# l13039968960/stm32H7-YOLO

Measured on AMD Instinct MI355X. Metric: images/sec int8 YOLO-face 56x56, higher is better.
Workload: dtype int8; 1 GPU; BASELINE configs[1]: batch=4096 int8 YOLO-face 56x56x3 frames per GPU, fused LDS-resident forward + GPU box decode; frames_per_gpu=4096, global_batch=4096, frame_bytes_in=9408, frame_bytes_out=882, input_batches_rotated=8, input_bytes_resident=308281344, kernel=yoloface56_fused<F=2,NW=8>, requant_rounding=ref, parallelism=single GPU, gather_every=1, collectives_issued=0, launch_streams=2

## Files before the change

stm32h7-yolo_amd/csrc/yf_kernels.hip.h:

```cpp
#include <hip/hip_runtime.h>
#include <stddef.h>
#include <stdint.h>
#include <type_traits>
#include "yf_tables.h"

#pragma clang diagnostic push
#pragma clang diagnostic ignored "-Wint-to-pointer-cast"
#if !defined(YF_LAB) || !defined(YF_LAUNDER)
#undef YF_LAUNDER
#define YF_LAUNDER 0
#endif
#define YF_ROW_SKEW 4
namespace YF_NS {

#ifndef YF_NOINLINE_STAGES
#define YF_STAGE_FN __device__ __forceinline__
#else
#define YF_STAGE_FN __device__ __attribute__((noinline))
#endif

typedef int v4i __attribute__((ext_vector_type(4)));
typedef short v2s __attribute__((ext_vector_type(2)));

#if !defined(YF_H0) || YF_H0 == 56
// ... 477 lines not shown
  for (int i = tid; i < F * IH * NCH * 5; i += NT) {
    const int cg = i % 5; int t = i / 5;
    const int k = t % NCH; t /= NCH;
    const int y = t % IH; const int f = t / IH;
    char* fbase = frames + f * B_T4::FS;
    const char* row = fbase + B_T4::at(y, 0) + 4 * cg;
    char* dst = fbase + B_HB::OFF + (y * OW) * 20 + 4 * cg;
    pool8_sweep<NO, B_T4::W - 1>(min(k * NO, OW - NO),
                                 [&](int x) { return lds_u32(row + x * B_T4::S); },
                                 [&](int ox, const SplitB& v) { *reinterpret_cast<uint32_t*>(dst + ox * 20) = v.merge(); });
  }
}
template <int F, int NT, bool STASH = false>
YF_STAGE_FN void pool8_v(char* frames, int tid) {
  constexpr int NO = 5, OW = B_HB::W, OH = B_T14::H, NCH = (OH + NO - 1) / NO;
  static_assert(OH >= NO, "column shorter than one sweep");
  for (int i = tid; i < F * OW * NCH * 5; i += NT) {
    const int cg = i % 5; int t = i / 5;
    const int k = t % NCH; t /= NCH;
    const int ox = t % OW; const int f = t / OW;
    char* fbase = frames + f * B_HB::FS;
    const char* col = fbase + B_HB::OFF + ox * 20 + 4 * cg;
    char* dst = fbase + B_T14::OFF + ox * B_T14::S + 4 * cg;
    pool8_sweep<NO, B_HB::H - 1>(min(k * NO, OH - NO),
                                 [&](int r) { return lds_u32(col + r * (OW * 20)); },
                                 [&](int oy, const SplitB& v) {
                                   *reinterpret_cast<uint32_t*>(dst + oy * (OW * B_T14::S)) = lut4_raw<YF_L_Q21>(v);
                                   if constexpr (STASH) *reinterpret_cast<uint32_t*>(dst + oy * (OW * B_T14::S) + YF_T14_CONV_BASE) = v.merge();
                                 });
  }
}

namespace v2 {
constexpr int LUT_B = YF_N_LUT * 256;
constexpr int JT = LUT_B, JT_B = 896;
constexpr int ZERO = JT + JT_B, ZERO_B = 640;
constexpr int SLOT0 = ZERO + ZERO_B, SLOT_B = 2816;
constexpr int slot(int cs) { return SLOT0 + (cs & 1) * SLOT_B; }
struct Lay56 {
  static constexpr int ZERO = v2::ZERO, JT = v2::JT, JT_BYTES = v2::JT_B;
  static constexpr int slot(int cs) { return v2::slot(cs); }
};
constexpr int max_block() { int m = 0; for (int i = 0; i < YF_N_CS; ++i) m = PLAN.vb_bytes[i] > m ? PLAN.vb_bytes[i] : m; return m; }
static_assert(max_block() <= SLOT_B && SLOT0 % 16 == 0 && SLOT_B % 16 == 0, "a constant block fits a ring slot");

typedef const __attribute__((address_space(3))) v4i* lds_v4i_ptr;
typedef const __attribute__((address_space(3))) v4u* lds_v4u_ptr;
typedef const __attribute__((address_space(3))) uint32_t* lds_u32_ptr;
typedef const __attribute__((address_space(3))) v2u* lds_u2_ptr;
__device__ __forceinline__ v4i lds_v4i(uint32_t a) { return *(lds_v4i_ptr)a; }
__device__ __forceinline__ v4u lds_v4u(uint32_t a) { return *(lds_v4u_ptr)a; }

template <int CS, class LAY = Lay56, int BYTES_ = -1>
__device__ __forceinline__ void fetch_consts(const uint8_t* __restrict__ tab, int wave, int lane) {
  constexpr int BYTES = BYTES_ >= 0 ? BYTES_ : PLAN.vb_bytes[CS], NCHUNK = (BYTES + 1023) / 1024;
  if (wave < NCHUNK) {
    asm volatile("" : "+v"(lane));
    const int off = wave * 1024 + lane * 16;
    if (off < BYTES) {
      const uint8_t* src = tab + PLAN.vb_off[CS] + off;
      const uint32_t dst = (uint32_t)(LAY::slot(CS) + wave * 1024);
      uint32_t keep;
      asm volatile("s_mov_b32 %0, m0\n\ts_mov_b32 m0, %2\n\ts_nop 0\n\tglobal_load_lds_dwordx4 %1, off\n\ts_mov_b32 m0, %0"
                   : "=&s"(keep) : "v"(src), "s"(dst) : "memory");
    }
  }
}

template <int W, int SH = (W > 32 ? 20 : 16)> struct DivW {
  static constexpr uint32_t M = ((1u << SH) + W - 1) / W;
  static constexpr bool ok() { for (uint32_t p = 0; p < 2048; ++p) if (((p * M) >> SH) != p / W) return false; return true; }
  static_assert(ok(), "multiply-shift division is exact on [0, 2048)");
  __device__ static __forceinline__ int div(int p) { return (int)(((uint32_t)p * M) >> SH); }
};

template <int EPI, int LUT_ID, int LA, int STASH_LUT = -1>
__device__ __forceinline__ void epilogue2(char* dstpix, const char* addpix, char* headpix, int chq, int hq, const int (&idx)[4], const AddK& ad,
                                          char* stashpix = nullptr) {
  if constexpr (EPI == EPI_LUT) {
    *reinterpret_cast<uint32_t*>(dstpix + chq) = join4(lutb<LUT_ID>(idx[0]), lutb<LUT_ID>(idx[1]), lutb<LUT_ID>(idx[2]), lutb<LUT_ID>(idx[3]));
    if constexpr (STASH_LUT >= 0) {
      if (stashpix) *reinterpret_cast<uint32_t*>(stashpix + chq) =
          join4(*(lds_u8_ptr)(uint32_t)(STASH_LUT + idx[0]), *(lds_u8_ptr)(uint32_t)(STASH_LUT + idx[1]),
                *(lds_u8_ptr)(uint32_t)(STASH_LUT + idx[2]), *(lds_u8_ptr)(uint32_t)(STASH_LUT + idx[3]));
    }
  } else if constexpr (EPI == EPI_RAW) {
    *reinterpret_cast<uint32_t*>(dstpix + chq) = join4(idx[0], idx[1], idx[2], idx[3]) ^ 0x80808080u;
  } else if constexpr (EPI == EPI_ADD) {
    typedef const __attribute__((address_space(3))) int* lds_i32_ptr;
    if (stashpix) *reinterpret_cast<uint32_t*>(stashpix + chq) = join4(idx[0], idx[1], idx[2], idx[3]) ^ 0x80808080u;
    const uint32_t o = lds_u32(addpix + chq) ^ 0x80808080u;
    v4i sum;
#pragma unroll
    for (int j = 0; j < 4; ++j)
      sum[j] = *(lds_i32_ptr)(uint32_t)(LA + 4 * ((o >> (8 * j)) & 255)) + *(lds_i32_ptr)(uint32_t)(LA + 1024 + 4 * idx[j]);
    int r[4];
    requant4<false>(sum, v4u{ad.mo2, ad.mo2, ad.mo2, ad.mo2}, v4u{ad.zro, ad.zro, ad.zro, ad.zro},
                    v4ul{ad.c64o, ad.c64o, ad.c64o, ad.c64o}, v4i{ad.rso, ad.rso, ad.rso, ad.rso}, r);
    *reinterpret_cast<uint32_t*>(dstpix + chq) = join4(r[0], r[1], r[2], r[3]) ^ 0x80808080u;
  } else {
    const uint32_t v = join4(idx[0], idx[1], idx[2], idx[3]) ^ 0x80808080u;
    uint16_t* dst = reinterpret_cast<uint16_t*>(headpix + hq);
    dst[0] = (uint16_t)v;
    if (hq + 2 < 18) dst[1] = (uint16_t)(v >> 16);
  }
}

template <int EPI, int LUT_ID, int LA>
__device__ __forceinline__ void epilogue2_half(char* dstpix, const char* addpix, int chq, const int (&idx)[2], const AddK& ad) {
  static_assert(EPI == EPI_LUT || EPI == EPI_RAW || EPI == EPI_ADD, "half passes: LUT, raw and residual-add epilogues");
  if constexpr (EPI == EPI_LUT) {
    *reinterpret_cast<uint32_t*>(dstpix + chq) = join2(lutb<LUT_ID>(idx[0]), lutb<LUT_ID>(idx[1]));
  } else if constexpr (EPI == EPI_RAW) {
    *reinterpret_cast<uint32_t*>(dstpix + chq) = join2(idx[0], idx[1]) ^ 0x8080u;
  } else {
    typedef const __attribute__((address_space(3))) int* lds_i32_ptr;
    const uint32_t o = lds_u32(addpix + chq) ^ 0x80808080u;
    v4i sum = {0, 0, 0, 0};
#pragma unroll
    for (int j = 0; j < 2; ++j)
      sum[j] = *(lds_i32_ptr)(uint32_t)(LA + 4 * ((o >> (8 * j)) & 255)) + *(lds_i32_ptr)(uint32_t)(LA + 1024 + 4 * idx[j]);
    int r[2];
    requant2<false>(sum, v4u{ad.mo2, ad.mo2, ad.mo2, ad.mo2}, v4u{ad.zro, ad.zro, ad.zro, ad.zro},
                    v4ul{ad.c64o, ad.c64o, ad.c64o, ad.c64o}, v4i{ad.rso, ad.rso, ad.rso, ad.rso}, r);
    *reinterpret_cast<uint32_t*>(dstpix + chq) = join2(r[0], r[1]) ^ 0x8080u;
  }
}
#if !defined(YF_LAB) || !defined(YF_CHUNK_UNROLL)
#undef YF_CHUNK_UNROLL
#define YF_CHUNK_UNROLL 0
#endif
#define YF_HALF_PASS 1

template <int F, int NW, int TPJ, int KS, int BW, class IN, class OUT, int OUT_CH0, int COUT, int EPI, int LUT_ID, class ADDB, int CS,
          int STASH_OFF = -1, int STASH_S = 0, int STASH_LUT = -1, class LAY = Lay56, int LA_ABS = -1>
YF_STAGE_FN void dense2_stage(char* frames, char* out_all, const uint8_t* __restrict__ tab, const AddK ad, int wave, int lane) {
  constexpr int NP = (COUT + 3) / 4, NCH = (NP + TPJ - 1) / TPJ;
  constexpr int P = IN::P, TOT = F * P;
  constexpr bool FRAME_TILES = P <= 64;
  constexpr int MT = FRAME_TILES ? F : (TOT + 63) / 64;
  constexpr int JOBS = NCH * MT, KROW = 16 * KS;
  constexpr int SLOT = LAY::slot(CS), WB = plan_wbytes(CS), PV = SLOT + WB, LA = LA_ABS >= 0 ? LA_ABS : PV + NP * (int)sizeof(yf_pass_v);
  static_assert(yf_cs_dense[CS] >= 0 && KROW == PLAN_KROW[yf_cs_dense[CS]] && NP == plan_passes(CS), "stage and constant block agree");
  static_assert((EPI == EPI_ADD) == (yf_cs_add[CS] >= 0), "residual-add tables travel with their stage");
  static_assert(OUT::P == P || EPI == EPI_HEAD || EPI == EPI_HEAD_LDS, "1x1 conv keeps the grid");
  static_assert(IN::FS == OUT::FS && IN::FS == ADDB::FS, "one frame stride per stage");
  static_assert(IN::S >= 16 * (KS - 1) + BW && (BW == 4 || BW == 8 || BW == 16), "the pixel vector must cover all k-steps");
  static_assert(IN::RS == IN::W && IN::PT == 0 && IN::PL == 0, "dense inputs are plain buffers");
  const int g = lane >> 4, c = lane & 15;
  const bool a_on = (c >> 2) == g;
  const uint32_t a_lane = a_on ? (uint32_t)(SLOT + (c & 3) * KROW) : (uint32_t)LAY::ZERO;
  const uint32_t a_step = a_on ? (uint32_t)(TPJ * 4 * KROW) : 0u;
  const uint8_t* sc = tab + PLAN.sb_off[CS];
  int in_c = 0, out_c = 0, add_c = 0, stash_c = 0;
  static_assert(STASH_OFF < 0 || EPI == EPI_ADD || (EPI == EPI_LUT && STASH_LUT >= 0), "a stash is the pre-add convolution output or a second LUT's view");
  if constexpr (FRAME_TILES) {
    const int p = min(lane, P - 1);
    in_c = IN::OFF + p * IN::S;
    if constexpr (EPI == EPI_HEAD || EPI == EPI_HEAD_LDS) out_c = p * 18;
    else if constexpr (OUT::RS == OUT::W && OUT::PT == 0 && OUT::PL == 0) out_c = OUT::OFF + p * OUT::S + OUT_CH0;
    else { const int y = DivW<OUT::W>::div(p); out_c = OUT::at(y, p - y * OUT::W) + OUT_CH0; }
    add_c = ADDB::OFF + p * ADDB::S;
    if constexpr (STASH_OFF >= 0) stash_c = STASH_OFF + p * STASH_S;
  }
  int j0, j1;
  job_range<JOBS, NW>(wave, j0, j1);
  auto run_chunk = [&](const int chunk, int mt, const int n) __attribute__((always_inline)) {
    v4i a[TPJ][KS];
    PassV pv[TPJ];
    PassS ksr[TPJ];
    const uint32_t a_addr = a_lane + (uint32_t)chunk * a_step;
#pragma unroll
    for (int t = 0; t < TPJ; ++t) {
      const int ps = chunk * TPJ + t;
#pragma unroll
      for (int ks = 0; ks < KS; ++ks) a[t][ks] = lds_v4i(a_addr + (uint32_t)(t * 4 * KROW + 16 * ks));
      pv[t].m2 = lds_v4u((uint32_t)(PV + ps * 32));
      pv[t].zr = lds_v4u((uint32_t)(PV + ps * 32 + 16));
      const uint8_t* s = sc + min(ps, NP - 1) * (int)sizeof(yf_pass_s);
      ksr[t] = PassS{*(cv4ul_ptr)(uintptr_t)s, *(cv4i_ptr)(uintptr_t)(s + 32)};
    }
    const int cq = chunk * TPJ * 4;
    const int out_cc = out_c + cq, add_cc = add_c + cq;
    for (int k = 0; k < n; ++k, ++mt) {
      const char* src; char* dstpix = nullptr; const char* addpix = nullptr; char* headpix = nullptr; char* stashpix = nullptr;
      if constexpr (FRAME_TILES) {
        char* fbase = frames + mt * IN::FS;
        src = fbase + in_c;
        dstpix = fbase + out_cc; addpix = fbase + add_cc;
        if constexpr (STASH_OFF >= 0) stashpix = fbase + stash_c + cq;
        if constexpr (EPI == EPI_HEAD) headpix = out_all + mt * OUT_FRAME_BYTES + out_c;
        if constexpr (EPI == EPI_HEAD_LDS) headpix = fbase + OUT::OFF + out_c;
      } else {
        const int q = min(mt * 64 + lane, TOT - 1);
        int f = 0;
#pragma unroll
        for (int i = 1; i < F; ++i) f += (q >= i * P) ? 1 : 0;
        const int p = q - f * P;
        char* fbase = frames + f * IN::FS;
        src = fbase + IN::OFF + p * IN::S;
        if constexpr (EPI == EPI_HEAD) headpix = out_all + f * OUT_FRAME_BYTES + p * 18;
        else if constexpr (EPI == EPI_HEAD_LDS) headpix = fbase + OUT::OFF + p * 18;
        else if constexpr (OUT::RS == OUT::W && OUT::PT == 0 && OUT::PL == 0) dstpix = fbase + cq + OUT::OFF + p * OUT::S + OUT_CH0;
        else { const int y = DivW<OUT::W>::div(p); dstpix = fbase + cq + OUT::at(y, p - y * OUT::W) + OUT_CH0; }
        if constexpr (EPI == EPI_ADD) addpix = fbase + cq + ADDB::OFF + p * ADDB::S;
        if constexpr (STASH_OFF >= 0) stashpix = fbase + cq + STASH_OFF + p * STASH_S;
      }
      v4i b[KS];
#pragma unroll
      for (int ks = 0; ks < KS - 1; ++ks) b[ks] = *reinterpret_cast<const v4i*>(src + 16 * ks);
      const char* last = src + 16 * (KS - 1);
      if constexpr (BW == 16) b[KS - 1] = *reinterpret_cast<const v4i*>(last);
      else if constexpr (BW == 8) { const int2 t2 = *reinterpret_cast<const int2*>(last); b[KS - 1] = v4i{t2.x, t2.y, any_value(), any_value()}; }
      else b[KS - 1] = v4i{*reinterpret_cast<const int*>(last), any_value(), any_value(), any_value()};
#pragma unroll
      for (int t = 0; t < TPJ; ++t) {
        const int ps = chunk * TPJ + t;
        if (ps < NP) {
          v4i acc = acc_init(pv[t].zr);
#pragma unroll
          for (int ks = 0; ks < KS; ++ks) acc = __builtin_amdgcn_mfma_i32_16x16x64_i8(a[t][ks], b[ks], acc, 0, 0, 0);
          constexpr bool HALF_L = YF_HALF_PASS && COUT % 4 == 2 && STASH_OFF < 0 && (EPI == EPI_LUT || EPI == EPI_RAW || EPI == EPI_ADD);
          const bool half = HALF_L && t == (NP - 1) % TPJ && ps == NP - 1;
          if (half) {
            if constexpr (HALF_L) {
              int idx2[2];
              requant2<true, DENSE_SIGNLESS, RQ_FP32>(acc, pv[t].m2, pv[t].zr, ksr[t].c64, ksr[t].rs, idx2);
              epilogue2_half<EPI, LUT_ID, LA>(dstpix, addpix, t * 4, idx2, ad);
            }
          } else {
            int idx[4];
            requant4<true, DENSE_SIGNLESS, RQ_FP32>(acc, pv[t].m2, pv[t].zr, ksr[t].c64, ksr[t].rs, idx);
            epilogue2<EPI, LUT_ID, LA, STASH_LUT>(dstpix, addpix, headpix, t * 4, ps * 4, idx, ad, stashpix);
          }
        }
      }
    }
  };
  if constexpr (NCH <= YF_CHUNK_UNROLL) {
#pragma unroll
    for (int chunk = 0; chunk < NCH; ++chunk) {
      const int lo = max(j0, chunk * MT), hi = min(j1, (chunk + 1) * MT);
      if (lo < hi) run_chunk(chunk, lo - chunk * MT, hi - lo);
    }
  } else {
    int chunk = (int)((uint32_t)j0 / (uint32_t)MT), mt = j0 - chunk * MT, left = j1 - j0;
    while (left > 0) {
      const int n = min(left, MT - mt);
      run_chunk(chunk, mt, n);
      left -= n; ++chunk; mt = 0;
    }
  }
}

template <int F, int NW, int CS, class IN = B_IN, class OUT = B_T1, class LAY = Lay56>
YF_STAGE_FN void conv1_2_stage(char* frames, const uint8_t* __restrict__ tab, int wave, int lane) {
  constexpr int P = OUT::P, W1 = OUT::W, RSW = IN::RS, TOT = F * P;
  constexpr int MT = (TOT + 63) / 64;
  constexpr int SLOT = LAY::slot(CS), WB = plan_wbytes(CS), PV = SLOT + WB;
  const int g = lane >> 4, c = lane & 15;
  const bool a_on = (c >> 2) == g;
  const uint32_t a_addr = a_on ? (uint32_t)(SLOT + (c & 3) * YF_CONV1_KROW) : (uint32_t)LAY::ZERO;
  const uint8_t* sc = tab + PLAN.sb_off[CS];
  v4i a[2][3];
  PassV pv[2];
#pragma unroll
  for (int ps = 0; ps < 2; ++ps) {
#pragma unroll
    for (int ks = 0; ks < 3; ++ks) a[ps][ks] = lds_v4i(a_addr + (uint32_t)(ps * 4 * YF_CONV1_KROW + 16 * ks));
    pv[ps].m2 = lds_v4u((uint32_t)(PV + ps * 32));
    pv[ps].zr = lds_v4u((uint32_t)(PV + ps * 32 + 16));
  }
  int j0, j1;
  job_range<MT, NW>(wave, j0, j1);
  const AddK ad = {};
  for (int mt = j0; mt < j1; ++mt) {
    const int q = min(mt * 64 + lane, TOT - 1);
    int f = 0;
#pragma unroll
    for (int i = 1; i < F; ++i) f += (q >= i * P) ? 1 : 0;
    const int p = q - f * P;
    const int oy = DivW<W1>::div(p), ox = p - oy * W1;
    char* fbase = frames + f * IN::FS;
    const uint32_t* src = reinterpret_cast<const uint32_t*>(fbase + IN::OFF) + (2 * oy * RSW + 2 * ox + 3);
    const v4i b0 = {(int)src[0], (int)src[1], (int)src[2], (int)src[RSW]};
    const v4i b1 = {(int)src[RSW + 1], (int)src[RSW + 2], (int)src[2 * RSW], (int)src[2 * RSW + 1]};
    const v4i b2 = {(int)src[2 * RSW + 2], any_value(), any_value(), any_value()};
    char* dstpix = fbase + OUT::at(oy, ox);
#pragma unroll
    for (int ps = 0; ps < 2; ++ps) {
      const uint8_t* s = sc + ps * (int)sizeof(yf_pass_s);
      const PassS k = PassS{*(cv4ul_ptr)(uintptr_t)s, *(cv4i_ptr)(uintptr_t)(s + 32)};
      v4i acc = acc_init(pv[ps].zr);
      acc = __builtin_amdgcn_mfma_i32_16x16x64_i8(a[ps][0], b0, acc, 0, 0, 0);
      acc = __builtin_amdgcn_mfma_i32_16x16x64_i8(a[ps][1], b1, acc, 0, 0, 0);
      acc = __builtin_amdgcn_mfma_i32_16x16x64_i8(a[ps][2], b2, acc, 0, 0, 0);
      int idx[4];
      requant4<true, DENSE_SIGNLESS, RQ_FP32>(acc, pv[ps].m2, pv[ps].zr, k.c64, k.rs, idx);
      epilogue2<EPI_LUT, YF_L_LEAKY2, 0>(dstpix, nullptr, nullptr, 4 * ps, 0, idx, ad);
    }
  }
}

template <int F, int STRIDE, int W, int H>
constexpr int dw_rows_per_lane() {
#if YF_H0 == 56
  return STRIDE == 1 && F == 2 && W == 28 && H == 28 ? 7 : STRIDE == 1 && F == 2 && W == 14 && H == 14 ? 2 : 1;
#else
  return 1;
#endif
}
template <int F, int STRIDE, class IN, class OUT>
struct DwGeo {
  static constexpr int W = OUT::W, H = OUT::H;
  static constexpr int R = dw_rows_per_lane<F, STRIDE, OUT::W, OUT::H>(), BR = 4 * R;
  static constexpr int FL = (W <= 8 && F % 2 == 0) ? 2 : 1;
  static constexpr int NSEG = (W + 15) / 16, NRB = (H + BR - 1) / BR, NFP = F / FL;
  static constexpr int JPG = NFP * NRB * NSEG;
  static_assert(OUT::RS == W && OUT::PT == 0 && OUT::PL == 0, "depthwise outputs are plain buffers");
  static_assert(IN::FS == OUT::FS, "one frame stride per stage");
  static_assert(H >= BR && (W >= 16 || W * FL <= 16), "tile shape");
  static_assert(R == 1 || (STRIDE == 1 && FL == 1), "row window: stride-1 stages, one frame per job");
  __device__ static __forceinline__ uint2 job(int jj) {
    const int fp = jj / (NRB * NSEG); int rem = jj - fp * (NRB * NSEG);
    const int rb = rem / NSEG, seg = rem - rb * NSEG;
    const int oy0 = min(rb * BR, H - BR);
    const int x0 = (W >= 16) ? min(seg * 16, W - 16) : 0;
    const int fb = fp * FL * IN::FS;
    return uint2{(uint32_t)(fb + IN::OFF + (oy0 * STRIDE) * IN::ROWB + x0 * STRIDE * IN::S), (uint32_t)(fb + OUT::OFF + (oy0 * W + x0) * OUT::S)};
  }
};
#if YF_H0 == 56
template <int F, bool BATCH>
struct JobTabs {
  typedef TailBufs<BATCH ? FRAME_STRIDE / 2 : FRAME_STRIDE> U;
  static constexpr int FT = BATCH ? 2 * F : F;
  static constexpr int JT_DW3 = 0;
  static constexpr int JT_DW10 = JT_DW3 + 8 * DwGeo<F, 1, B_T1, B_T2>::JPG;
  static constexpr int JT_DW15 = JT_DW10 + 8 * DwGeo<F, 2, B_T4, B_T6>::JPG;
  static constexpr int JT_DW27 = JT_DW15 + 8 * DwGeo<F, 1, B_T8, B_T9>::JPG;
  static constexpr int JT_DW32 = JT_DW27 + 8 * DwGeo<FT, 2, typename U::T15, typename U::T17>::JPG;
  static constexpr int END = JT_DW32 + 8 * DwGeo<FT, 1, typename U::T19, typename U::T20>::JPG;
  static_assert(END <= JT_B, "job tables fit");
};
#endif
template <class B, bool RING, int F>
struct HaloGeo {
  static constexpr int HR = B::H + B::PT + (RING ? 1 : 0), WR = B::RS;
  static constexpr int NPIX = RING ? (2 * WR + 2 * (HR - 2)) : (WR + HR - 1);
  static constexpr int N = F * NPIX;
  static_assert(B::S % 4 == 0 && B::OFF % 4 == 0 && B::FS % 4 == 0, "dword pixels");
  __device__ static __forceinline__ uint32_t entry(int i) {
    const int f = i / NPIX, k = i - f * NPIX;
    int r, c;
    if constexpr (RING) {
      if (k < WR) { r = 0; c = k; }
      else if (k < 2 * WR) { r = HR - 1; c = k - WR; }
      else { const int m = k - 2 * WR; r = 1 + (m >> 1); c = (m & 1) ? WR - 1 : 0; }
    } else {
      if (k < WR) { r = 0; c = k; } else { r = 1 + (k - WR); c = 0; }
    }
    return (uint32_t)(f * B::FS + B::OFF + r * B::ROWB + c * B::S);
  }
};
#if YF_H0 == 56
template <int F, bool BATCH>
struct HaloTabs {
  typedef TailBufs<BATCH ? FRAME_STRIDE / 2 : FRAME_STRIDE> U;
  static constexpr int FT = BATCH ? 2 * F : F;
  typedef HaloGeo<B_T1, true, F> G1; typedef HaloGeo<B_T4, false, F> G4; typedef HaloGeo<B_T8, true, F> G8;
  typedef HaloGeo<B_T15, false, F> G15; typedef HaloGeo<typename U::T19, true, FT> G19;
  static constexpr int H_T1 = 0, H_T4 = H_T1 + 2 * G1::N, H_T8 = H_T4 + 2 * G4::N, H_T15 = H_T8 + 2 * G8::N, H_T19 = H_T15 + 2 * G15::N;
  static constexpr int BYTES = (H_T19 + 2 * G19::N + 15) & ~15;
};
constexpr int HT = SLOT0 + 2 * SLOT_B;
template <int F, bool BATCH> constexpr int pre_bytes() { return HT + HaloTabs<F, BATCH>::BYTES; }
template <class G, int HOFF, int NT>
__device__ __forceinline__ void build_halotab(char* smem, int tid) {
  for (int i = tid; i < G::N; i += NT) *reinterpret_cast<uint16_t*>(smem + HT + HOFF + 2 * i) = (uint16_t)(G::entry(i) >> 2);
}
template <class B, class G, int HOFF>
YF_STAGE_FN void fill_halo_t(char* frames, int zp, int tid) {
  typedef const __attribute__((address_space(3))) uint16_t* lds_u16_ptr;
  if (tid < G::N) {
    const uint32_t v = (uint32_t)(zp & 255) * 0x01010101u;
    char* p = frames + 4u * (uint32_t)*(lds_u16_ptr)(uint32_t)(HT + HOFF + 2 * tid);
    if constexpr (B::S % 8 == 0 && B::OFF % 8 == 0 && B::FS % 8 == 0) {
#pragma unroll
      for (int d = 0; d < B::S / 8; ++d) *reinterpret_cast<uint2*>(p + 8 * d) = uint2{v, v};
    } else {
#pragma unroll
      for (int d = 0; d < B::S / 4; ++d) *reinterpret_cast<uint32_t*>(p + 4 * d) = v;
    }
  }
}
#endif

template <int F, int STRIDE, class IN, class OUT, int JTOFF, class LAY = Lay56>
__device__ __forceinline__ void fill_jobtab(char* smem, int tid) {
  typedef DwGeo<F, STRIDE, IN, OUT> G;
  static_assert(JTOFF % 8 == 0 && JTOFF + G::JPG * 8 <= LAY::JT_BYTES, "job table in bounds");
  if (tid < G::JPG) *reinterpret_cast<uint2*>(smem + LAY::JT + JTOFF + 8 * tid) = G::job(tid);
}

template <int F, int NW, int STRIDE, class IN, class OUT, int C, int LUT_ID, int CS, int JTOFF, class LAY = Lay56>
YF_STAGE_FN void dw2_stage(char* frames, const uint8_t* __restrict__ tab, int wave, int lane) {
  typedef DwGeo<F, STRIDE, IN, OUT> G;
  constexpr int W = G::W, FL = G::FL, JPG = G::JPG;
  constexpr int NG = (C + 3) / 4, JOBS = NG * JPG;
  constexpr int DROW = STRIDE * IN::ROWB;
  constexpr int TS = IN::S, TR = IN::ROWB;
  constexpr int SLOT = LAY::slot(CS);
  static_assert(yf_cs_dw[CS] >= 0 && NG == plan_passes(CS), "stage and constant block agree");
  const int g = lane >> 4, c = lane & 15;
  const int fl = (FL == 2) ? (c >> 3) : 0;
  const int xl = (FL == 2) ? min(c & 7, W - 1) : min(c, W - 1);
  const char* lane_in = frames + fl * IN::FS + g * G::R * DROW + xl * STRIDE * IN::S;
  char* lane_out = frames + fl * IN::FS + (g * G::R * W + xl) * OUT::S;
  const bool a_on = (c >> 2) == g;
  const uint32_t a_lane = a_on ? (uint32_t)(SLOT + 4 * (c & 3)) : (uint32_t)LAY::ZERO;
  const uint32_t a_step = a_on ? (uint32_t)YF_DWV_GROUP_BYTES : 0u;
  const uint8_t* sc = tab + PLAN.sb_off[CS];
  int j, j1;
  job_range<JOBS, NW>(wave, j, j1);
  int cg = (int)((uint32_t)j / (uint32_t)JPG), jj = j - cg * JPG, left = j1 - j;
  while (left > 0) {
    const uint32_t wa = a_lane + (uint32_t)cg * a_step;
    v4i a0, a1, a2 = {0, 0, 0, 0};
    a0 = v4i{(int)*(lds_u32_ptr)(wa), (int)*(lds_u32_ptr)(wa + 16), (int)*(lds_u32_ptr)(wa + 32), (int)*(lds_u32_ptr)(wa + 48)};
    a1 = v4i{(int)*(lds_u32_ptr)(wa + 64), (int)*(lds_u32_ptr)(wa + 80), (int)*(lds_u32_ptr)(wa + 96), (int)*(lds_u32_ptr)(wa + 112)};
    a2[0] = (int)*(lds_u32_ptr)(wa + 128);
    PassV pv;
    pv.m2 = lds_v4u((uint32_t)(SLOT + cg * YF_DWV_GROUP_BYTES + 144));
    pv.zr = lds_v4u((uint32_t)(SLOT + cg * YF_DWV_GROUP_BYTES + 160));
    const uint8_t* s = sc + cg * (int)sizeof(yf_pass_s);
    const PassS k = PassS{*(cv4ul_ptr)(uintptr_t)s, *(cv4i_ptr)(uintptr_t)(s + 32)};
    const char* lin = lane_in + 4 * cg;
    char* lout = lane_out + 4 * cg;
    auto entry = [&](int job) { return *(lds_u2_ptr)(uint32_t)(LAY::JT + JTOFF + 8 * min(job, JPG - 1)); };
    auto taps = [&](const v2u e, v4i& b0, v4i& b1, v4i& b2, char*& dst) {
      const char* src = lin + e[0];
      b0[0] = (int)lds_u32(src);               b0[1] = (int)lds_u32(src + TS);          b0[2] = (int)lds_u32(src + 2 * TS);
      b0[3] = (int)lds_u32(src + TR);          b1[0] = (int)lds_u32(src + TR + TS);     b1[1] = (int)lds_u32(src + TR + 2 * TS);
      b1[2] = (int)lds_u32(src + 2 * TR);      b1[3] = (int)lds_u32(src + 2 * TR + TS); b2[0] = (int)lds_u32(src + 2 * TR + 2 * TS);
      dst = lout + e[1];
    };
    auto conv = [&](const v4i& b0, const v4i& b1, const v4i& b2) {
      v4i acc = acc_init(pv.zr);
      acc = __builtin_amdgcn_mfma_i32_16x16x64_i8(a0, b0, acc, 0, 0, 0);
      acc = __builtin_amdgcn_mfma_i32_16x16x64_i8(a1, b1, acc, 0, 0, 0);
      return __builtin_amdgcn_mfma_i32_16x16x64_i8(a2, b2, acc, 0, 0, 0);
    };
    auto finish = [&](const v4i& acc, char* dst) {
      if (YF_HALF_PASS && C % 4 == 2 && cg == NG - 1) {
        int idx2[2];
        requant2<true, false, RQ_FP32>(acc, pv.m2, pv.zr, k.c64, k.rs, idx2);
        *reinterpret_cast<uint32_t*>(dst) = join2(lutb<LUT_ID>(idx2[0]), lutb<LUT_ID>(idx2[1]));
      } else {
        int idx[4];
        requant4<true, false, RQ_FP32>(acc, pv.m2, pv.zr, k.c64, k.rs, idx);
        *reinterpret_cast<uint32_t*>(dst) = join4(lutb<LUT_ID>(idx[0]), lutb<LUT_ID>(idx[1]), lutb<LUT_ID>(idx[2]), lutb<LUT_ID>(idx[3]));
      }
    };
    const int n = min(left, JPG - jj);
    if constexpr (G::R > 1) {
      const v4i ar[3] = {v4i{a0[0], a0[1], a0[2], 0}, v4i{a0[3], a1[0], a1[1], 0}, v4i{a1[2], a1[3], a2[0], 0}};
      for (int i = 0; i < n; ++i) {
        const v2u e = entry(jj + i);
        const char* src = lin + e[0];
        char* dst = lout + e[1];
        auto row = [&](int r) {
          const char* p = src + r * TR;
          return v4i{(int)lds_u32(p), (int)lds_u32(p + TS), (int)lds_u32(p + 2 * TS), any_value()};
        };
        v4i w0 = row(0), w1 = row(1);
#pragma unroll
        for (int y = 0; y < G::R; ++y) {
          const v4i w2 = row(y + 2);
          v4i acc = acc_init(pv.zr);
          acc = __builtin_amdgcn_mfma_i32_16x16x64_i8(ar[0], w0, acc, 0, 0, 0);
          acc = __builtin_amdgcn_mfma_i32_16x16x64_i8(ar[1], w1, acc, 0, 0, 0);
          acc = __builtin_amdgcn_mfma_i32_16x16x64_i8(ar[2], w2, acc, 0, 0, 0);
          finish(acc, dst + y * W * OUT::S);
          w0 = w1; w1 = w2;
        }
      }
      left -= n; ++cg; jj = 0;
      continue;
    }
    int i = 0;
    v2u e0 = entry(jj), e1 = entry(jj + 1);
    for (; i + 1 < n; i += 2) {
      v4i p0, p1, p2 = {0, any_value(), any_value(), any_value()}, q0, q1, q2 = {0, any_value(), any_value(), any_value()};
      char *dp, *dq;
      taps(e0, p0, p1, p2, dp);
      taps(e1, q0, q1, q2, dq);
      e0 = entry(jj + i + 2); e1 = entry(jj + i + 3);
      const v4i ap = conv(p0, p1, p2);
      const v4i aq = conv(q0, q1, q2);
      finish(ap, dp);
      finish(aq, dq);
    }
    if (i < n) {
      v4i b0, b1, b2 = {0, any_value(), any_value(), any_value()};
      char* dst;
      taps(e0, b0, b1, b2, dst);
      finish(conv(b0, b1, b2), dst);
    }
    left -= n; ++cg; jj = 0;
  }
}
template <int FT> constexpr int pool25_waves() { return (FT * 42 + 63) / 64; }
template <int FT, class T15, class T30, bool STASH = false>
YF_STAGE_FN void pool25_cols(char* frames, int item) {
  static_assert(T15::W == 14 && T15::H == 14 && T30::W == 7 && T15::FS == T30::FS, "pool_25 geometry");
  const int t = DivW<6>::div(item), cg = item - 6 * t;
  const int f = DivW<7>::div(t), ox = t - 7 * f;
  if (f >= FT) return;
  char* fbase = frames + f * T15::FS;
  const char* base = fbase + T15::at(0, 0) + 4 * cg;
  constexpr int S = T15::S, ROW = T15::ROWB;
  const int c0 = max(2 * ox - 1, 0) * S, c1 = 2 * ox * S, c2 = c1 + S, c3 = min(2 * ox + 2, 13) * S;
  auto hrow = [&](int r) {
    const char* p = base + r * ROW;
    return SplitB(lds_u32(p + c0)).mx(SplitB(lds_u32(p + c1))).mx(SplitB(lds_u32(p + c2))).mx(SplitB(lds_u32(p + c3)));
  };
  char* dst = fbase + T30::OFF + ox * T30::S + 4 * cg;
  SplitB prev = hrow(0);
#pragma unroll
  for (int oy = 0; oy < 7; ++oy) {
    SplitB next = hrow(2 * oy + 1);
    if (2 * oy + 2 <= 13) next = next.mx(hrow(2 * oy + 2));
    const SplitB mxv = prev.mx(next);
    *reinterpret_cast<uint32_t*>(dst + oy * (7 * T30::S)) = lut4_raw<YF_L_Q45>(mxv);
    if constexpr (STASH) *reinterpret_cast<uint32_t*>(dst + oy * (7 * T30::S) + 24) = mxv.merge();
    prev = next;
  }
}
}
#ifndef YF_GENERIC
#include "yf_fused56.hip.h"
#else
#ifdef YF_LAB
#include "yf_lab_layerwise.hip.h"
#endif
#include "yf_band160.hip.h"
#endif

}
#pragma clang diagnostic pop
```

Baseline: 31.05 million images/s.

## Extend depthwise row-window walk to stride-2 stages with frame groups per wave

Generalizes the per-lane row window in depthwise stages so stride-2 layers (14x14 and 7x7 outputs) also walk multiple output rows per lane, reusing the shared input row between consecutive stride-2 windows. Lane groups can now cover separate frames (FG) as well as row blocks, which changes job geometry and lane addressing. The aim is fewer jobs, fewer job-table loads and fewer redundant LDS row loads per output. In exchange, the unrolled loops are longer and register pressure rises, and rows can overlap when BR exceeds H (the clamped seg_row), so some work is recomputed.

```diff
diff --git a/stm32h7-yolo_amd/csrc/yf_kernels.hip.h b/stm32h7-yolo_amd/csrc/yf_kernels.hip.h
--- a/stm32h7-yolo_amd/csrc/yf_kernels.hip.h
+++ b/stm32h7-yolo_amd/csrc/yf_kernels.hip.h
@@ -803,31 +803,35 @@
   }
 }
 
+struct DwWalk { int R, FG; };
 template <int F, int STRIDE, int W, int H>
-constexpr int dw_rows_per_lane() {
+constexpr DwWalk dw_rows_per_lane() {
 #if YF_H0 == 56
-  return STRIDE == 1 && F == 2 && W == 28 && H == 28 ? 7 : STRIDE == 1 && F == 2 && W == 14 && H == 14 ? 2 : 1;
-#else
-  return 1;
-#endif
+  if (STRIDE == 1 && F == 2 && W == 28 && H == 28) return DwWalk{7, 1};
+  if (STRIDE == 1 && F == 2 && W == 14 && H == 14) return DwWalk{2, 1};
+  if (STRIDE == 2 && F == 2 && W == 14 && H == 14) return DwWalk{7, 2};
+  if (STRIDE == 2 && F == 4 && W == 7 && H == 7) return DwWalk{4, 2};
+#endif
+  return DwWalk{1, 1};
 }
 template <int F, int STRIDE, class IN, class OUT>
 struct DwGeo {
   static constexpr int W = OUT::W, H = OUT::H;
-  static constexpr int R = dw_rows_per_lane<F, STRIDE, OUT::W, OUT::H>(), BR = 4 * R;
+  static constexpr DwWalk WK = dw_rows_per_lane<F, STRIDE, OUT::W, OUT::H>();
+  static constexpr int R = WK.R, FG = WK.FG, RG = 4 / FG, BR = RG * R;
   static constexpr int FL = (W <= 8 && F % 2 == 0) ? 2 : 1;
-  static constexpr int NSEG = (W + 15) / 16, NRB = (H + BR - 1) / BR, NFP = F / FL;
+  static constexpr int NSEG = (W + 15) / 16, NRB = (H + BR - 1) / BR, NFP = F / (FL * FG);
   static constexpr int JPG = NFP * NRB * NSEG;
   static_assert(OUT::RS == W && OUT::PT == 0 && OUT::PL == 0, "depthwise outputs are plain buffers");
   static_assert(IN::FS == OUT::FS, "one frame stride per stage");
-  static_assert(H >= BR && (W >= 16 || W * FL <= 16), "tile shape");
-  static_assert(R == 1 || (STRIDE == 1 && FL == 1), "row window: stride-1 stages, one frame per job");
+  static_assert((H >= BR || (R > 1 && H >= R)) && (W >= 16 || W * FL <= 16) && F % (FL * FG) == 0 && RG * FG == 4, "tile shape");
+  __device__ static __forceinline__ int seg_row(int rs) { return BR > H ? min(rs * R, H - R) : rs * R; }
   __device__ static __forceinline__ uint2 job(int jj) {
     const int fp = jj / (NRB * NSEG); int rem = jj - fp * (NRB * NSEG);
     const int rb = rem / NSEG, seg = rem - rb * NSEG;
-    const int oy0 = min(rb * BR, H - BR);
+    const int oy0 = BR > H ? 0 : min(rb * BR, H - BR);
     const int x0 = (W >= 16) ? min(seg * 16, W - 16) : 0;
-    const int fb = fp * FL * IN::FS;
+    const int fb = fp * FL * FG * IN::FS;
     return uint2{(uint32_t)(fb + IN::OFF + (oy0 * STRIDE) * IN::ROWB + x0 * STRIDE * IN::S), (uint32_t)(fb + OUT::OFF + (oy0 * W + x0) * OUT::S)};
   }
 };
@@ -916,8 +920,9 @@
   const int g = lane >> 4, c = lane & 15;
   const int fl = (FL == 2) ? (c >> 3) : 0;
   const int xl = (FL == 2) ? min(c & 7, W - 1) : min(c, W - 1);
-  const char* lane_in = frames + fl * IN::FS + g * G::R * DROW + xl * STRIDE * IN::S;
-  char* lane_out = frames + fl * IN::FS + (g * G::R * W + xl) * OUT::S;
+  const int fr = fl + FL * (g / G::RG), row0 = G::seg_row(g % G::RG);
+  const char* lane_in = frames + fr * IN::FS + row0 * DROW + xl * STRIDE * IN::S;
+  char* lane_out = frames + fr * IN::FS + (row0 * W + xl) * OUT::S;
   const bool a_on = (c >> 2) == g;
   const uint32_t a_lane = a_on ? (uint32_t)(SLOT + 4 * (c & 3)) : (uint32_t)LAY::ZERO;
   const uint32_t a_step = a_on ? (uint32_t)YF_DWV_GROUP_BYTES : 0u;
@@ -977,13 +982,15 @@
         v4i w0 = row(0), w1 = row(1);
 #pragma unroll
         for (int y = 0; y < G::R; ++y) {
-          const v4i w2 = row(y + 2);
+          if constexpr (STRIDE == 2) { if (y > 0) w1 = row(2 * y + 1); }
+          const v4i w2 = row(STRIDE * y + 2);
           v4i acc = acc_init(pv.zr);
           acc = __builtin_amdgcn_mfma_i32_16x16x64_i8(ar[0], w0, acc, 0, 0, 0);
           acc = __builtin_amdgcn_mfma_i32_16x16x64_i8(ar[1], w1, acc, 0, 0, 0);
           acc = __builtin_amdgcn_mfma_i32_16x16x64_i8(ar[2], w2, acc, 0, 0, 0);
           finish(acc, dst + y * W * OUT::S);
-          w0 = w1; w1 = w2;
+          if constexpr (STRIDE == 2) w0 = w2;
+          else { w0 = w1; w1 = w2; }
         }
       }
       left -= n; ++cg; jj = 0;
```

New measurement: 31.65 million images/s, median of 6. 1.9% higher.
